# rhinempi/Reflexiv

Measured on AMD Instinct MI355X. Metric: k-mers/sec (extract+count+filter; wall-clock to final contigs beside it), higher is better.
Workload: dtype u64; 1 GPU; synthetic 5 Gbp in all (5 Gbp per GPU x 1), E.coli-like genome 4640000 bp (1078x), PE150, k=31, -cover 30, 0.5% substitutions; reads_per_gpu=33333334, kmer_instances_per_gpu=4000000080, distinct_kmers=352952250, kmers_kept=4639950, parallelism=1 GPU

## Files before the change

### reflexiv_amd/csrc/rfx_count_sk.hip

```cpp
#include "rfx_internal.h"
#include "rfx_device.h"
#include "rfx_count.h"
#include <algorithm>
#include <cmath>

using namespace rfxd;
using namespace rfxc;

namespace {


constexpr int SKT = 1024;

__device__ __forceinline__ uint32_t mmer_key(uint32_t canon) { return __umul24(canon, 0x9E3779u) + canon; }

template <int W, bool RUNLOOP, int SEG = 16, class F>
__device__ __forceinline__ void seg_runs(const ReadSrc &s, int nk_r, int sgm, const uint64_t (&w)[3], F &&emit,
                                         uint64_t *hi_out, uint64_t *lo_out, uint32_t *wm_lds = nullptr, uint32_t *nx_out = nullptr) {
    static_assert(SEG == 16 || SEG == 32, "segment");
    constexpr int PK = SEG;
    constexpr bool MERGE = SEG == 32;
    static_assert(!MERGE || RUNLOOP, "the merged cut walks the run-start bits");
    constexpr int NM = PK + W - 1;
    static_assert(NM + SK_M - 1 <= 64, "the segment's bases lie in (hi, lo)");
    const int p0 = sgm * PK;
    int v = nk_r - p0;
    v = v > PK ? PK : v;
    if constexpr (MERGE) {
        v = v < 0 ? 0 : v;
        if (!__any(v > 0)) return;
    } else if (v <= 0) return;
    const int sh = 2 * ((s.fc + p0) & 31);
    const uint64_t hi = sh ? (w[0] << sh) | (w[1] >> (64 - sh)) : w[0];
    const uint64_t lo = sh ? (w[1] << sh) | (w[2] >> (64 - sh)) : w[1];
    *hi_out = hi; *lo_out = lo;
    constexpr int M2 = 2 * SK_M;
    const uint32_t mmask = (1u << M2) - 1;
    uint32_t val[NM];
    static_assert(SK_M == 13 && NM <= 50, "positions below");
    const uint64_t rhi = revcomp(lo, 32), rlo = revcomp(hi, 32);
    const uint32_t FW[4] = {(uint32_t)(hi >> 32), (uint32_t)hi, (uint32_t)(lo >> 32), (uint32_t)lo};
    const uint32_t RW[4] = {(uint32_t)(rhi >> 32), (uint32_t)rhi, (uint32_t)(rlo >> 32), (uint32_t)rlo};
    auto cut = [&](const uint32_t (&Wd)[4], const int pos) __attribute__((always_inline)) -> uint32_t {
        const int wi = pos >> 4, off = 2 * (pos & 15);
        if (off + M2 <= 32) return (Wd[wi] >> (32 - M2 - off)) & mmask;
        return __builtin_amdgcn_alignbit(Wd[wi], Wd[wi < 3 ? wi + 1 : 3], 32 - off) >> (32 - M2);
    };
#pragma unroll
    for (int j = 0; j < NM; j++) {
        const uint32_t fm = cut(FW, j), rm = cut(RW, 64 - SK_M - j);
        val[j] = mmer_key(fm < rm ? fm : rm);
    }
    uint32_t wm[PK];
    if constexpr (W >= PK - 1) {
#pragma unroll
        for (int j = W - 2; j >= 0; j--) val[j] = val[j] < val[j + 1] ? val[j] : val[j + 1];
#pragma unroll
        for (int j = W + 1; j < NM; j++) val[j] = val[j] < val[j - 1] ? val[j] : val[j - 1];
        wm[0] = val[0];
#pragma unroll
        for (int i = 1; i < PK; i++) wm[i] = val[i] < val[W + i - 1] ? val[i] : val[W + i - 1];
    } else {
        uint32_t sfx[NM], pfx[NM];
#pragma unroll
        for (int j = NM - 1; j >= 0; j--)
            sfx[j] = (j % W == W - 1 || j == NM - 1) ? val[j] : (val[j] < sfx[j + 1] ? val[j] : sfx[j + 1]);
#pragma unroll
        for (int j = 0; j < NM; j++) pfx[j] = (j % W == 0) ? val[j] : (val[j] < pfx[j - 1] ? val[j] : pfx[j - 1]);
#pragma unroll
        for (int i = 0; i < PK; i++) wm[i] = sfx[i] < pfx[i + W - 1] ? sfx[i] : pfx[i + W - 1];
    }
    if constexpr (!RUNLOOP) {
        uint32_t cur = wm[0];
        int start = 0;
#pragma unroll
        for (int i = 1; i < PK; i++) {
            if (i < v && (wm[i] != cur || (PK > 16 && i - start == 16))) {
                emit(start, i - start, cur);
                cur = wm[i]; start = i;
            }
        }
        emit(start, v - start, cur);
        return;
    }
    uint32_t starts = 1u;
#pragma unroll
    for (int i = 1; i < PK; i++) starts |= (uint32_t)(wm[i] != wm[i - 1]) << i;
    const uint32_t vmask = v ? 0xffffffffu >> (32 - v) : 0u;
    starts &= vmask;
    if constexpr (PK > 16) {
        uint32_t cov = starts;
        cov |= cov << 1; cov |= cov << 2; cov |= cov << 4; cov |= cov << 8;
        const uint32_t unc = ~cov & vmask;
        starts |= unc & (0u - unc);
    }
    int vend = v;
    if constexpr (MERGE) {
        const int lane = (int)(threadIdx.x & 63);
        const uint32_t rest = starts & (starts - 1);
        const int b = !v ? 0 : rest ? __ffs((int)rest) - 1 : v;
        const int t = v == PK ? __clz((int)starts) + 1 : 0;
        const uint32_t hk = wm[0], tk = wm[PK - 1];
        const uint32_t hk_n = (uint32_t)__shfl_down((int)hk, 1);
        const uint32_t pk_n = (uint32_t)__shfl_down((int)(((uint32_t)(lo >> 32) & 0xFFFFFFC0u) | (uint32_t)b), 1);
        const uint32_t tk_p = (uint32_t)__shfl_up((int)tk, 1);
        const int t_p = __shfl_up(t, 1);
        const bool next_same = lane < 63 && sgm + 1 < s.segs, prev_same = lane > 0 && sgm > 0;
        const int b_n = (int)(pk_n & 31u);
        if (nx_out) *nx_out = next_same ? pk_n & 0xFFFFFFC0u : 0u;
        if (next_same && t > 0 && b_n > 0 && tk == hk_n) vend = v + (16 - t < b_n ? 16 - t : b_n);
        if (prev_same && t_p > 0 && b > 0 && tk_p == hk) {
            const int a = 16 - t_p < b ? 16 - t_p : b;
            if (a > 0) starts = (starts & ~1u) | (a < b ? 1u << a : 0u);
        }
    }
    if (wm_lds) {
#pragma unroll
        for (int i = 0; i < PK; i++) wm_lds[i * SKT + threadIdx.x] = wm[i];
    }
    uint32_t m0 = wm[0], m1 = wm[1], m2 = wm[2], m3 = wm[3], m4 = wm[4], m5 = wm[5], m6 = wm[6], m7 = wm[7], m8 = wm[8],
             m9 = wm[9], m10 = wm[10], m11 = wm[11], m12 = wm[12], m13 = wm[13], m14 = wm[14], m15 = wm[15];
    if (!wm_lds)
        asm("" : "+v"(m0), "+v"(m1), "+v"(m2), "+v"(m3), "+v"(m4), "+v"(m5), "+v"(m6), "+v"(m7), "+v"(m8), "+v"(m9), "+v"(m10),
                 "+v"(m11), "+v"(m12), "+v"(m13), "+v"(m14), "+v"(m15));
    constexpr int UP = PK > 16 ? 16 : 0;
    uint32_t n0 = wm[UP + 0], n1 = wm[UP + 1], n2 = wm[UP + 2], n3 = wm[UP + 3], n4 = wm[UP + 4], n5 = wm[UP + 5], n6 = wm[UP + 6],
             n7 = wm[UP + 7], n8 = wm[UP + 8], n9 = wm[UP + 9], n10 = wm[UP + 10], n11 = wm[UP + 11], n12 = wm[UP + 12],
             n13 = wm[UP + 13], n14 = wm[UP + 14], n15 = wm[UP + 15];
    if (!wm_lds && PK > 16)
        asm("" : "+v"(n0), "+v"(n1), "+v"(n2), "+v"(n3), "+v"(n4), "+v"(n5), "+v"(n6), "+v"(n7), "+v"(n8), "+v"(n9), "+v"(n10),
                 "+v"(n11), "+v"(n12), "+v"(n13), "+v"(n14), "+v"(n15));
    while (starts) {
        const int i0 = __ffs((int)starts) - 1;
        starts &= starts - 1;
        const int i1 = starts ? __ffs((int)starts) - 1 : vend;
        uint32_t key;
        if (wm_lds) {
            key = wm_lds[i0 * SKT + threadIdx.x];
        } else {
            const bool b0 = i0 & 1, b1 = i0 & 2, b2 = i0 & 4, b3 = i0 & 8;
            const uint32_t a0 = b0 ? m1 : m0, a1 = b0 ? m3 : m2, a2 = b0 ? m5 : m4, a3 = b0 ? m7 : m6, a4 = b0 ? m9 : m8,
                           a5 = b0 ? m11 : m10, a6 = b0 ? m13 : m12, a7 = b0 ? m15 : m14;
            const uint32_t c0 = b1 ? a1 : a0, c1 = b1 ? a3 : a2, c2 = b1 ? a5 : a4, c3 = b1 ? a7 : a6;
            const uint32_t d0 = b2 ? c1 : c0, d1 = b2 ? c3 : c2;
            key = b3 ? d1 : d0;
            if constexpr (PK > 16) {
                const uint32_t e0 = b0 ? n1 : n0, e1 = b0 ? n3 : n2, e2 = b0 ? n5 : n4, e3 = b0 ? n7 : n6, e4 = b0 ? n9 : n8,
                               e5 = b0 ? n11 : n10, e6 = b0 ? n13 : n12, e7 = b0 ? n15 : n14;
                const uint32_t f0 = b1 ? e1 : e0, f1 = b1 ? e3 : e2, f2 = b1 ? e5 : e4, f3 = b1 ? e7 : e6;
                const uint32_t g0 = b2 ? f1 : f0, g1 = b2 ? f3 : f2;
                const uint32_t ku = b3 ? g1 : g0;
                key = (i0 & 16) ? ku : key;
            }
        }
        emit(i0, i1 - i0, key);
    }
}

__device__ __forceinline__ uint64_t mmer_hash64(uint32_t canon) { return kmer_hash((uint64_t)canon); }

__device__ __forceinline__ unsigned sk_digit(uint32_t canon, const Level &lv) {
    const uint64_t h = mmer_hash64(canon);
    if (lv.n_owners > 0) {
        const unsigned o = (unsigned)__umul64hi(h, (uint64_t)lv.n_owners);
        return lv.sub_bits ? (o << lv.sub_bits) | ((uint32_t)((h << OWNER_BITS) >> 32) >> (32 - lv.sub_bits)) : o;
    }
    return rec_digit((uint32_t)((h << OWNER_BITS) >> 32), 0, lv.bits);
}

constexpr int SKD = 8;

template <int W, bool DESC, bool WIDE = false>
__global__ __launch_bounds__(SKT) void k_sk_hist(ReadSrc s, Level lv, uint64_t *__restrict__ blockhist,
                                                 uint32_t *__restrict__ desc) {
    __shared__ uint32_t h[1 << MAX_BITS];
    __shared__ uint32_t wmcol[DESC ? PK * SKT : 1];
    const int nb = lv.n_owners > 0 ? lv.n_owners : (1 << lv.bits);
    for (int i = threadIdx.x; i < nb; i += SKT) h[i] = 0;
    __syncthreads();
    const int64_t stride = (int64_t)gridDim.x * SKT;
    const int64_t dq = stride / s.segs;
    const int dr = (int)(stride - dq * s.segs);
    int64_t g = (int64_t)blockIdx.x * SKT + threadIdx.x;
    SegPos q;
    q.r = g / s.segs;
    q.sgm = (int)(g - q.r * s.segs);
    for (; g < s.n_threads; g += stride) {
        uint64_t w[3], hi, lo;
        seg_load(s, q, w);
        if constexpr (DESC) {
            uint32_t mask = 0, nr = 0;
            uint32_t own[2] = {0, 0};
            seg_runs<W, true>(s, read_nk<WIDE>(s, q.r), q.sgm, w, [&](int i0, int, uint32_t canon) {
                const uint64_t h64 = mmer_hash64(canon);
                const uint32_t hdr = (uint32_t)((h64 << OWNER_BITS) >> 32);
                const unsigned d = lv.n_owners > 0 ? (unsigned)__umul64hi(h64, (uint64_t)lv.n_owners) : rec_digit(hdr, 0, lv.bits);
                atomicAdd(&h[d], 1u);
                if (nr < (uint32_t)SKD) {
                    desc[(int64_t)(1 + nr) * s.n_threads + g] = hdr;
                    if (nr < 4) own[0] |= d << (8 * nr); else own[1] |= d << (8 * (nr - 4));
                }
                mask |= 1u << i0; nr++;
            }, &hi, &lo, wmcol);
            desc[g] = mask | (nr << 16);
            if (lv.n_owners > 0) {
                desc[(int64_t)(1 + SKD) * s.n_threads + g] = own[0];
                desc[(int64_t)(2 + SKD) * s.n_threads + g] = own[1];
            }
        } else {
            seg_runs<W, false>(s, read_nk<WIDE>(s, q.r), q.sgm, w, [&](int, int, uint32_t canon) { atomicAdd(&h[sk_digit(canon, lv)], 1u); }, &hi, &lo);
        }
        q.r += dq; q.sgm += dr;
        if (q.sgm >= s.segs) { q.sgm -= s.segs; q.r++; }
    }
    __syncthreads();
    for (int i = threadIdx.x; i < nb; i += SKT) blockhist[(int64_t)i * gridDim.x + blockIdx.x] = h[i];
}

constexpr int SKB = 8, SKA = 4;
template <int W, bool DESC, bool WIDE = false>
__global__ __launch_bounds__(SKT, WIDE ? 4 : 8) void k_sk_scatter(ReadSrc s, Level lv, const uint64_t *__restrict__ scanned,
                                                              std::conditional_t<WIDE, WRec, Rec> *__restrict__ out,
                                                              const uint32_t *__restrict__ desc) {
    using RT = std::conditional_t<WIDE, WRec, Rec>;
    extern __shared__ __attribute__((aligned(32))) unsigned char sk_smem[];
    const int nb = lv.n_owners > 0 ? lv.n_owners : (1 << lv.bits);
#define buf ((RT *)sk_smem)
#define tail ((unsigned long long *)(sk_smem + (size_t)nb * SKB * sizeof(RT)))
#define head (tail + nb)
    for (int i = threadIdx.x; i < nb; i += SKT) tail[i] = head[i] = scanned[(int64_t)i * gridDim.x + blockIdx.x];
    __syncthreads();
    auto drain = [&](bool final) __attribute__((always_inline)) {
        for (int d = threadIdx.x / SKB; d < nb; d += SKT / SKB) {
            const int j = threadIdx.x % SKB;
            const unsigned long long h = head[d], t = tail[d];
            unsigned long long e, nh;
            if (t - h > (unsigned long long)SKB) { e = h + SKB; nh = t; }
            else {
                e = final ? t : (t & ~(unsigned long long)(SKA - 1));
                if (e < h) e = h;
                nh = e;
            }
            const unsigned long long g = h + j;
            if (g < e) out[g] = buf[(size_t)d * SKB + (g & (SKB - 1))];
            if (j == 0) head[d] = nh;
        }
    };
    const int64_t stride = (int64_t)gridDim.x * SKT;
    const int64_t dq = stride / s.segs;
    const int dr = (int)(stride - dq * s.segs);
    const int64_t g0 = (int64_t)blockIdx.x * SKT;
    int64_t g = g0 + threadIdx.x;
    SegPos q;
    q.r = g / s.segs;
    q.sgm = (int)(g - q.r * s.segs);
    for (int64_t gb = g0; gb < s.n_threads; gb += stride, g += stride) {
        if (g < s.n_threads) {
            uint64_t w[3], hi = 0, lo = 0;
            seg_load(s, q, w);
            auto put = [&](int i0, int n, uint32_t hdr, unsigned d) __attribute__((always_inline)) {
                RT r;
                if constexpr (WIDE) {
                    const uint64_t *gw = s.words + q.r * s.wpr;
                    const int p = s.fc - s.wfl + q.sgm * PK + i0;
                    const int wi = p >> 5, sft = 2 * (p & 31), last = s.wpr - 1;
                    const uint64_t a0 = gw[wi < last ? wi : last], a1 = gw[wi + 1 < last ? wi + 1 : last];
                    const uint64_t a2 = gw[wi + 2 < last ? wi + 2 : last], a3 = gw[wi + 3 < last ? wi + 3 : last];
                    r.b0 = sft ? (a0 << sft) | (a1 >> (64 - sft)) : a0;
                    r.b1 = sft ? (a1 << sft) | (a2 >> (64 - sft)) : a1;
                    r.b2 = sft ? (a2 << sft) | (a3 >> (64 - sft)) : a2;
                    r.hd = ((uint64_t)(n - 1) << 32) | (uint64_t)hdr;
                } else {
                    const int sft = 2 * i0;
                    r.w0 = sft ? (hi << sft) | (lo >> (64 - sft)) : hi;
                    r.w1 = ((lo << sft) & 0xFFFFFFF000000000ULL) | ((uint64_t)(n - 1) << 32) | (uint64_t)hdr;
                }
                const unsigned long long pos = atomicAdd(&tail[d], 1ULL);
                if (pos - head[d] < (unsigned long long)SKB) buf[(size_t)d * SKB + (pos & (SKB - 1))] = r;
                else out[pos] = r;
            };
            auto recompute = [&]() __attribute__((always_inline)) {
                seg_runs<W, true>(s, read_nk<WIDE>(s, q.r), q.sgm, w, [&](int i0, int n, uint32_t canon) {
                    const uint64_t h = mmer_hash64(canon);
                    const unsigned d = lv.n_owners > 0 ? (unsigned)__umul64hi(h, (uint64_t)lv.n_owners)
                                                       : rec_digit((uint32_t)((h << OWNER_BITS) >> 32), 0, lv.bits);
                    put(i0, n, (uint32_t)((h << OWNER_BITS) >> 32), d);
                }, &hi, &lo);
            };
            if constexpr (DESC) {
                const uint32_t m = desc[g];
                const uint32_t nr = m >> 16;
                if (nr > (uint32_t)SKD) {
                    recompute();
                } else if (nr) {
                    const int p0 = q.sgm * PK;
                    int v = read_nk<WIDE>(s, q.r) - p0;
                    v = v > PK ? PK : v;
                    const int sh = 2 * ((s.fc + p0) & 31);
                    hi = sh ? (w[0] << sh) | (w[1] >> (64 - sh)) : w[0];
                    lo = sh ? (w[1] << sh) | (w[2] >> (64 - sh)) : w[1];
                    uint32_t hd[SKD];
#pragma unroll
                    for (int r = 0; r < SKD; r++) hd[r] = (uint32_t)r < nr ? desc[(int64_t)(1 + r) * s.n_threads + g] : 0u;
                    uint32_t own[2] = {0, 0};
                    if (lv.n_owners > 0) {
                        own[0] = desc[(int64_t)(1 + SKD) * s.n_threads + g];
                        own[1] = desc[(int64_t)(2 + SKD) * s.n_threads + g];
                    }
                    uint32_t starts = m & 0xffffu;
#pragma unroll
                    for (int r = 0; r < SKD; r++) {
                        if (starts) {
                            const int i0 = __ffs((int)starts) - 1;
                            starts &= starts - 1;
                            const int i1 = starts ? __ffs((int)starts) - 1 : v;
                            put(i0, i1 - i0, hd[r], lv.n_owners > 0 ? (own[r >> 2] >> (8 * (r & 3))) & 255u : rec_digit(hd[r], 0, lv.bits));
                        }
                    }
                }
            } else {
                recompute();
            }
            q.r += dq; q.sgm += dr;
            if (q.sgm >= s.segs) { q.sgm -= s.segs; q.r++; }
        }
        __syncthreads();
        drain(false);
        __syncthreads();
    }
    drain(true);
}
#undef buf
#undef tail
#undef head

constexpr int OSE_MIN = 64, OSE_MAX = 256;
constexpr int OS_CSTRIDE = 16;
constexpr int OS_MAXG = 512;
constexpr int OS_HOLES = 3;
struct OneSweep {
    const uint64_t *reg_start;
    const uint32_t *reg_cap;
    unsigned long long *cursor;
    uint64_t *holes;
    int *overflow;
    uint64_t total;
    unsigned long long *tile_counter;
    uint32_t ose, ose_shift;
};

template <int W, int SEG = 16, bool WIDE = false>
__global__ __launch_bounds__(SKT) void k_sk_sample_hist(ReadSrc s, Level lv, int sample, unsigned long long *__restrict__ hist) {
    __shared__ uint32_t h[1 << MAX_BITS];
    const int nb = 1 << lv.bits;
    for (int i = threadIdx.x; i < nb; i += SKT) h[i] = 0;
    __syncthreads();
    const int64_t ntile = (s.n_threads + SKT - 1) / SKT;
    for (int64_t T = (int64_t)blockIdx.x * sample; T < ntile; T += (int64_t)gridDim.x * sample) {
        const int64_t g = T * SKT + threadIdx.x;
        const bool in = g < s.n_threads;
        SegPos q{0, 0};
        int nk_r = 0;
        uint64_t w[3] = {0, 0, 0}, hi, lo;
        if (in) {
            q.r = g / s.segs;
            q.sgm = (int)(g - q.r * s.segs);
            seg_load<SEG>(s, q, w);
            nk_r = read_nk<WIDE>(s, q.r);
        }
        if (SEG == 32 || in)
            seg_runs<W, SEG == 32, SEG>(s, nk_r, q.sgm, w, [&](int, int, uint32_t canon) { atomicAdd(&h[sk_digit(canon, lv)], 1u); }, &hi, &lo);
    }
    __syncthreads();
    for (int i = threadIdx.x; i < nb; i += SKT) if (h[i]) atomicAdd(&hist[i], (unsigned long long)h[i]);
}

__global__ __launch_bounds__(1024) void k_plan_regions(const unsigned long long *__restrict__ hist, int nb, double scale, int G, int cap_pct,
                                                       double tiles,
                                                       uint64_t *__restrict__ reg_start, uint32_t *__restrict__ reg_cap,
                                                       unsigned long long *__restrict__ cursor, unsigned long long *__restrict__ totals) {
    __shared__ uint64_t caps[1 << MAX_BITS];
    __shared__ unsigned long long busiest;
    __shared__ uint32_t ose_s;
    const int d = threadIdx.x;
    if (d == 0) busiest = 0;
    __syncthreads();
    if (d < nb) atomicMax(&busiest, hist[d]);
    __syncthreads();
    if (d == 0) {
        const double per_tile = (double)busiest * scale / tiles;
        ose_s = per_tile <= 16.0 ? 64u : per_tile <= 32.0 ? 128u : per_tile <= 64.0 ? 256u : 0u;
    }
    __syncthreads();
    const uint32_t E = ose_s ? ose_s : OSE_MIN;
    if (d < nb) {
        const double c = (double)hist[d];
        const double est = c * scale;
        double room = (est + 6.0 * scale * sqrt(c + 1.0) + est / 64.0 + 1024.0) * (double)cap_pct / 100.0;
        uint64_t cap = (uint64_t)room + (uint64_t)G * OS_HOLES * E;
        cap = (cap + E - 1) / E * E;
        if (cap > 0xFFFFFF00ULL) cap = 0xFFFFFF00ULL / E * E;
        caps[d] = cap;
        reg_cap[d] = (uint32_t)cap;
    }
    __syncthreads();
    if (threadIdx.x == 0) {
        uint64_t at = 0;
        for (int i = 0; i < nb; i++) { reg_start[i] = at; cursor[(size_t)i * OS_CSTRIDE] = at; at += caps[i]; }
        reg_start[nb] = at;
        totals[0] = at + E;
        totals[1] = 0;
        totals[2] = ose_s;
    }
}

template <int SEG, bool WIDE> struct OsGeo {
    static constexpr int T = SEG > 16 && !WIDE ? 512 : SKT;
};
template <int W, bool WIDE = false, int SEG = 16>
__global__ __launch_bounds__((OsGeo<SEG, WIDE>::T), 4) void k_sk_onesweep(ReadSrc s, Level lv, OneSweep os,
                                                               std::conditional_t<WIDE, WRec, Rec> *__restrict__ out) {
    using RT = std::conditional_t<WIDE, WRec, Rec>;
    constexpr int SKT = OsGeo<SEG, WIDE>::T;
    extern __shared__ __attribute__((aligned(32))) unsigned char sk_smem[];
    const int nb = 1 << lv.bits;
#define buf ((RT *)sk_smem)
#define tail ((uint32_t *)(sk_smem + (size_t)nb * SKB * sizeof(RT)))
#define head (tail + nb)
#define cstart (tail + 2 * nb)
#define cbase (tail + 3 * nb)
#define nbase (tail + 4 * nb)
#define pbase (tail + 5 * nb)
    constexpr uint32_t DUMP = 0xFFFFFFFFu;
    const uint32_t OSE = os.ose, OSH = os.ose_shift;
    const uint64_t dump_at = os.total - OSE;
    auto extent_of = [&](unsigned long long b) __attribute__((always_inline)) -> uint32_t {
        return b + OSE <= dump_at ? (uint32_t)(b >> OSH) : DUMP;
    };
    auto grab = [&](int d) __attribute__((always_inline)) -> uint32_t {
        return extent_of(atomicAdd(&os.cursor[(size_t)d * OS_CSTRIDE], (unsigned long long)OSE));
    };
    auto phys = [&](uint32_t v, uint32_t cs, uint32_t cb, uint32_t nx) __attribute__((always_inline)) -> uint64_t {
        const uint32_t o = v - cs;
        const uint32_t b = o < (uint32_t)OSE ? cb : nx;
        return (b == DUMP ? dump_at : (uint64_t)b << OSH) + (o & (OSE - 1));
    };
    constexpr uint32_t NONE = 0xFFFFFFFEu;
    for (int i = threadIdx.x; i < nb; i += SKT) {
        tail[i] = 0; head[i] = 0; cstart[i] = 0;
        cbase[i] = grab(i);
        nbase[i] = grab(i);
        pbase[i] = grab(i);
    }
    __syncthreads();
    constexpr int LPB = SEG > 16 || WIDE ? 4 : SKB;
    auto drain = [&](bool final) __attribute__((always_inline)) {
#pragma nounroll
        for (int d = threadIdx.x / LPB; d < nb; d += SKT / LPB) {
            const int j = threadIdx.x % LPB;
            const uint32_t h = head[d], t = tail[d], cs = cstart[d], cb = cbase[d], nx = nbase[d];
            uint32_t e, nh;
            if (t - h > (uint32_t)SKB) { e = h + SKB; nh = t; }
            else {
                e = final ? t : (t & ~(uint32_t)(SKA - 1));
                if (e < h) e = h;
                nh = e;
            }
#pragma unroll
            for (int q = 0; q < SKB / LPB; q++) {
                const uint32_t g = h + j + q * LPB;
                if (g < e) l2_store_stream(out + phys(g, cs, cb, nx), buf[(size_t)d * SKB + (g & (SKB - 1))]);
            }
            if (j == 0) {
                head[d] = nh;
                if (nh - cs >= (uint32_t)OSE) {
                    const uint32_t b2 = pbase[d];
                    cstart[d] = cs + OSE; cbase[d] = nx; nbase[d] = final && b2 == NONE ? DUMP : b2; pbase[d] = NONE;
                }
            }
        }
    };
    __shared__ long long tile_lds[2];
    const int64_t ntile = (s.n_threads + SKT - 1) / SKT;
    const int my_d = (int)threadIdx.x;
    int64_t T = blockIdx.x;
    auto fetch = [&](int64_t tile, SegPos &q, int &nk_r, uint64_t (&w)[3]) __attribute__((always_inline)) {
        const int64_t g = tile * SKT + threadIdx.x;
        const int64_t gc = g < s.n_threads ? g : s.n_threads - 1;
        q.r = gc / s.segs;
        q.sgm = (int)(gc - q.r * s.segs);
        seg_load<SEG>(s, q, w);
        nk_r = read_nk<WIDE>(s, q.r);
    };
    int64_t T1 = (int64_t)gridDim.x + blockIdx.x;
    SegPos qn{0, 0};
    int nkn = 0;
    uint64_t wn[3] = {0, 0, 0};
    if (T < ntile) fetch(T, qn, nkn, wn);
    asm volatile("" : "+v"(wn[0]), "+v"(wn[1]), "+v"(wn[2]), "+v"(nkn));
    for (int rnd = 0; T < ntile; rnd++) {
        const bool in = T * SKT + threadIdx.x < s.n_threads;
        SegPos q{in ? qn.r : 0, in ? qn.sgm : 0};
        int nk_r = in ? nkn : 0;
        uint64_t w[3] = {in ? wn[0] : 0, in ? wn[1] : 0, in ? wn[2] : 0}, hi = 0, lo = 0;
        uint32_t past = 0;
        unsigned long long t_raw = 0, req_raw = 0;
        const bool ask = my_d < nb && pbase[my_d] == NONE;
        if (ask) req_raw = atomicAdd(&os.cursor[(size_t)my_d * OS_CSTRIDE], (unsigned long long)OSE);
        fetch(T1, qn, nkn, wn);
        if (threadIdx.x == SKT - 1) t_raw = atomicAdd(os.tile_counter, 1ULL);
        if (SEG == 32 || in) {
            seg_runs<W, true, SEG>(s, nk_r, q.sgm, w, [&](int i0, int n, uint32_t canon) {
                const uint64_t hh = mmer_hash64(canon);
                const uint32_t hdr = (uint32_t)((hh << OWNER_BITS) >> 32);
                const unsigned d = lv.n_owners > 0 ? (((unsigned)__umul64hi(hh, (uint64_t)lv.n_owners) << lv.sub_bits) | (hdr >> (32 - lv.sub_bits)))
                                                   : rec_digit(hdr, 0, lv.bits);
                RT r;
                if constexpr (WIDE) {
                    const uint64_t *gw = s.words + q.r * s.wpr;
                    const int p = s.fc - s.wfl + q.sgm * SEG + i0;
                    const int wi = p >> 5, sft = 2 * (p & 31), last = s.wpr - 1;
                    const uint64_t a0 = gw[wi < last ? wi : last], a1 = gw[wi + 1 < last ? wi + 1 : last];
                    const uint64_t a2 = gw[wi + 2 < last ? wi + 2 : last], a3 = gw[wi + 3 < last ? wi + 3 : last];
                    r.b0 = sft ? (a0 << sft) | (a1 >> (64 - sft)) : a0;
                    r.b1 = sft ? (a1 << sft) | (a2 >> (64 - sft)) : a1;
                    r.b2 = sft ? (a2 << sft) | (a3 >> (64 - sft)) : a2;
                    r.hd = ((uint64_t)(n - 1) << 32) | (uint64_t)hdr;
                } else {
                    const uint32_t d0 = (uint32_t)(hi >> 32), d1 = (uint32_t)hi, d2 = (uint32_t)(lo >> 32), d3 = (uint32_t)lo;
                    const uint32_t e0 = d0 >> 1, e1 = __builtin_amdgcn_alignbit(d0, d1, 1), e2 = __builtin_amdgcn_alignbit(d1, d2, 1);
                    const uint32_t e3 = __builtin_amdgcn_alignbit(d2, d3, 1), e4 = __builtin_amdgcn_alignbit(d3, past, 1);
                    const bool up = i0 >= 16;
                    const uint32_t a0 = up ? e1 : e0, a1 = up ? e2 : e1, a2 = up ? e3 : e2, a3 = up ? e4 : e3;
                    const uint32_t sh = 31u - 2u * ((uint32_t)i0 & 15u);
                    const uint32_t w0h = __builtin_amdgcn_alignbit(a0, a1, sh), w0l = __builtin_amdgcn_alignbit(a1, a2, sh);
                    const uint32_t w1h = (__builtin_amdgcn_alignbit(a2, a3, sh) & 0xFFFFFFF0u) | (uint32_t)(n - 1);
                    r.w0 = ((uint64_t)w0h << 32) | w0l;
                    r.w1 = ((uint64_t)w1h << 32) | (uint64_t)hdr;
                }
                const uint32_t pos = atomicAdd(&tail[d], 1u);
                if (pos - head[d] < (uint32_t)SKB) buf[(size_t)d * SKB + (pos & (SKB - 1))] = r;
                else {
                    const uint32_t cs = cstart[d];
                    if (pos - cs < 2u * OSE) out[phys(pos, cs, cbase[d], nbase[d])] = r;
                    else { os.overflow[0] = 1; os.overflow[1] = 1; }
                }
            }, &hi, &lo, nullptr, &past);
        }
        asm volatile("" : "+v"(wn[0]), "+v"(wn[1]), "+v"(wn[2]), "+v"(nkn), "+v"(t_raw), "+v"(req_raw));
        if (threadIdx.x == SKT - 1) tile_lds[rnd & 1] = 2LL * (long long)gridDim.x + (long long)t_raw;
        if (ask) pbase[my_d] = extent_of(req_raw);
        __syncthreads();
        drain(false);
        T = T1;
        T1 = tile_lds[rnd & 1];
        __syncthreads();
    }
    drain(true);
    __syncthreads();
    for (int d = threadIdx.x; d < nb; d += SKT) {
        const uint32_t used = tail[d] - cstart[d], cb = cbase[d], nx = nbase[d], px = pbase[d];
        uint64_t *hl = os.holes + ((size_t)d * gridDim.x + blockIdx.x) * OS_HOLES;
        hl[0] = cb != DUMP && used < OSE ? ((((uint64_t)cb << OSH) + used) << 16) | (uint64_t)(OSE - used) : 0;
        hl[1] = nx != DUMP ? (((uint64_t)nx << OSH) << 16) | (uint64_t)OSE : 0;
        hl[2] = px != DUMP && px != NONE ? (((uint64_t)px << OSH) << 16) | (uint64_t)OSE : 0;
    }
}
#undef buf
#undef tail
#undef head
#undef cstart
#undef cbase
#undef nbase
#undef pbase

constexpr int FH_T = 1024;
template <class RT>
__global__ __launch_bounds__(FH_T) void k_fix_holes(OneSweep os, int G, RT *__restrict__ out, uint64_t *__restrict__ seg_begin,
                                                   uint64_t *__restrict__ seg_end, unsigned long long *__restrict__ totals) {
    constexpr int NHMAX = 2048;
    static_assert(NHMAX >= OS_HOLES * OS_MAXG && NHMAX % FH_T == 0, "holes per bucket");
    constexpr int NWMAX = NHMAX * OSE_MAX / 32;
    __shared__ uint32_t hstart[NHMAX], hoff[NHMAX + 1];
    __shared__ uint32_t bitmap[NWMAX];
    __shared__ uint32_t wsum[FH_T / 64];
    const int d = blockIdx.x;
    const int NH = OS_HOLES * G;
    const uint64_t base = os.reg_start[d];
    const unsigned long long alloc = os.cursor[(size_t)d * OS_CSTRIDE] - base;
    if (alloc > (unsigned long long)os.reg_cap[d]) {
        if (threadIdx.x == 0) { seg_begin[d] = base; seg_end[d] = base; *os.overflow = 1; }
        return;
    }
    auto block_excl_scan = [&](uint32_t v, uint32_t *total) __attribute__((always_inline)) -> uint32_t {
        const int lane = threadIdx.x & 63, wave = threadIdx.x >> 6;
        uint32_t x = v;
#pragma unroll
        for (int o = 1; o < 64; o <<= 1) { const uint32_t y = __shfl_up(x, o, 64); if (lane >= o) x += y; }
        if (lane == 63) wsum[wave] = x;
        __syncthreads();
        uint32_t b = 0, tot = 0;
        for (int i = 0; i < FH_T / 64; i++) { const uint32_t sv = wsum[i]; if (i < wave) b += sv; tot += sv; }
        __syncthreads();
        *total = tot;
        return b + x - v;
    };
    constexpr int HPT = NHMAX / FH_T;
    uint32_t hs[HPT], hl[HPT];
    uint32_t mine = 0;
#pragma unroll
    for (int r = 0; r < HPT; r++) {
        const int t = threadIdx.x * HPT + r;
        const uint64_t x = t < NH ? os.holes[(size_t)d * NH + t] : 0;
        hl[r] = (uint32_t)(x & 0xFFFFu);
        hs[r] = hl[r] ? (uint32_t)((x >> 16) - base) : 0u;
        mine += hl[r];
    }
    uint32_t H;
    block_excl_scan(mine, &H);
    const uint32_t size = (uint32_t)alloc - H;
    const uint32_t nw = (H + 31) / 32;
    const uint32_t wpt = (nw + FH_T - 1) / FH_T;
    for (uint32_t i = threadIdx.x; i < nw; i += FH_T) bitmap[i] = 0;
    __syncthreads();
    uint32_t fill[HPT], fsum = 0;
#pragma unroll
    for (int r = 0; r < HPT; r++) {
        fill[r] = hs[r] < size ? (hs[r] + hl[r] <= size ? hl[r] : size - hs[r]) : 0u;
        fsum += fill[r];
        for (uint32_t p = hs[r] + fill[r]; p < hs[r] + hl[r]; p++) atomicOr(&bitmap[(p - size) >> 5], 1u << ((p - size) & 31));
    }
    uint32_t F;
    uint32_t fo = block_excl_scan(fsum, &F);
#pragma unroll
    for (int r = 0; r < HPT; r++) {
        const int t = threadIdx.x * HPT + r;
        hstart[t] = hs[r]; hoff[t] = fo; fo += fill[r];
    }
    if (threadIdx.x == 0) hoff[NHMAX] = F;
    __syncthreads();
    auto valid_word = [&](uint32_t w) __attribute__((always_inline)) -> uint32_t {
        if (w >= nw) return 0u;
        const uint32_t lim = H - w * 32 >= 32 ? 0xFFFFFFFFu : (1u << (H - w * 32)) - 1u;
        return ~bitmap[w] & lim;
    };
    uint32_t vsum = 0;
    for (uint32_t r = 0; r < wpt; r++) vsum += (uint32_t)__popc(valid_word(threadIdx.x * wpt + r));
    uint32_t V;
    uint32_t vo = block_excl_scan(vsum, &V);
    for (uint32_t r = 0; r < wpt; r++) {
        const uint32_t w = threadIdx.x * wpt + r;
        uint32_t m = valid_word(w);
        while (m) {
            const int b = __ffs((int)m) - 1;
            m &= m - 1;
            const uint32_t i = vo++;
            if (i < F) {
                int lo = 0, hi = NHMAX;
                while (hi - lo > 1) { const int mid = (lo + hi) >> 1; if (hoff[mid] <= i) lo = mid; else hi = mid; }
                out[base + hstart[lo] + (i - hoff[lo])] = out[base + size + w * 32 + b];
            }
        }
    }
    if (threadIdx.x == 0) {
        seg_begin[d] = base; seg_end[d] = base + size;
        atomicAdd(&totals[1], (unsigned long long)size);
        if (V != F) *os.overflow = 2;
    }
}

}

namespace rfx {

#define RFX_SK_W_CASES(X) X(9) X(10) X(11) X(12) X(13) X(14) X(15) X(16) X(17) X(18)
template <bool DESC, bool WIDE = false, class... Args>
static int launch_sk_hist(rfx_ctx *ctx, int W, dim3 grid, Args... args) {
    if constexpr (WIDE) {
        if (W == 18) RFX_LAUNCH((k_sk_hist<18, DESC, true>), grid, dim3(SKT), 0, args...);
        else RFX_LAUNCH((k_sk_hist<19, DESC, true>), grid, dim3(SKT), 0, args...);
        return RFX_OK;
    }
    switch (W) {
#define X(w) case w: RFX_LAUNCH((k_sk_hist<w, DESC>), grid, dim3(SKT), 0, args...); break;
        RFX_SK_W_CASES(X)
#undef X
        default: RFX_LAUNCH((k_sk_hist<19, DESC>), grid, dim3(SKT), 0, args...); break;
    }
    return RFX_OK;
}

template <int W, bool DESC, bool WIDE, class... Args>
static int launch_sk_scatter_w(rfx_ctx *ctx, dim3 grid, size_t lds, Args... args) {
    RFX_HIP(hipFuncSetAttribute((const void *)k_sk_scatter<W, DESC, WIDE>, hipFuncAttributeMaxDynamicSharedMemorySize, (int)lds));
    RFX_LAUNCH((k_sk_scatter<W, DESC, WIDE>), grid, dim3(SKT), lds, args...);
    return RFX_OK;
}
template <bool DESC, bool WIDE, class... Args>
static int launch_sk_scatter(rfx_ctx *ctx, int W, dim3 grid, size_t lds, Args... args) {
    if constexpr (WIDE) {
        if (W == 18) return launch_sk_scatter_w<18, DESC, true>(ctx, grid, lds, args...);
        return launch_sk_scatter_w<19, DESC, true>(ctx, grid, lds, args...);
    } else {
        switch (W) {
#define X(w) case w: return launch_sk_scatter_w<w, DESC, false>(ctx, grid, lds, args...);
            RFX_SK_W_CASES(X)
#undef X
            default: return launch_sk_scatter_w<19, DESC, false>(ctx, grid, lds, args...);
        }
    }
}

template <bool WIDE>
int records_from_reads(rfx_ctx *ctx, const ReadSrc &rsrc, const Level &lv, bool use_ws, int ws_slot,
                       std::conditional_t<WIDE, WRec, Rec> *d_dst, int64_t cap_dst, uint64_t *d_seg_off,
                       std::conditional_t<WIDE, WRec, Rec> **out_recs, int64_t *n_recs,
                       const char *hn, const char *pn) {
    using Rec = std::conditional_t<WIDE, WRec, ::Rec>;
    const int nb = lv.n_owners > 0 ? lv.n_owners : (1 << lv.bits);
    const int W = rsrc.k - SK_M + 1;
    const size_t sk_lds = (size_t)nb * (SKB * sizeof(Rec) + 16);
    const int per_cu = sk_lds <= 80 * 1024 ? 8 : 1;
    const unsigned G = (unsigned)std::max<int64_t>(1, std::min<int64_t>(ceil_div(rsrc.n_threads, SKT), (int64_t)ctx->num_cu * per_cu));
    DevBuf bh, scanned;
    RFX_ALLOC(bh, uint64_t, (size_t)nb * G);
    RFX_ALLOC(scanned, uint64_t, (size_t)nb * G + 1);
    uint32_t *desc = nullptr;
    const bool want_desc = lv.n_owners <= 64 && count_tuning().sk_desc;
    if (want_desc) desc = (uint32_t *)ctx->ws_get(use_ws && ws_slot == 1 ? 0 : 1, (size_t)(3 + SKD) * 4 * (size_t)rsrc.n_threads);
    {
        ScopedTimer t(ctx, hn);
        if (desc) RFX_TRY((launch_sk_hist<true, WIDE>(ctx, W, dim3(G), rsrc, lv, bh.as<uint64_t>(), desc)));
        else RFX_TRY((launch_sk_hist<false, WIDE>(ctx, W, dim3(G), rsrc, lv, bh.as<uint64_t>(), (uint32_t *)nullptr)));
    }
    RFX_TRY(exclusive_scan_u64(ctx, bh.as<uint64_t>(), scanned.as<uint64_t>(), (int64_t)nb * G));
    RFX_TRY(bin_offsets(ctx, scanned.as<uint64_t>(), nb, (int64_t)G, d_seg_off));
    uint64_t R = 0;
    RFX_HIP(hipMemcpyAsync(&R, scanned.as<uint64_t>() + (size_t)nb * G, 8, hipMemcpyDeviceToHost, ctx->stream));
    RFX_TRY(sync_checked(ctx));
    *n_recs = (int64_t)R;
    Rec *dst = d_dst;
    if (use_ws) {
        dst = (Rec *)ctx->ws_get(ws_slot, (size_t)R * sizeof(Rec));
        if (!dst) { ctx->last_error = "workspace allocation failed"; return RFX_E_HIP; }
    } else if (!dst || (int64_t)R > cap_dst) {
        return RFX_E_CAP;
    }
    {
        ScopedTimer t(ctx, pn);
        if (desc) RFX_TRY((launch_sk_scatter<true, WIDE>(ctx, W, dim3(G), sk_lds, rsrc, lv, scanned.as<uint64_t>(), dst, (const uint32_t *)desc)));
        else RFX_TRY((launch_sk_scatter<false, WIDE>(ctx, W, dim3(G), sk_lds, rsrc, lv, scanned.as<uint64_t>(), dst, (const uint32_t *)nullptr)));
    }
    *out_recs = dst;
    return RFX_OK;
}

template <bool WIDE>
int records_onesweep(rfx_ctx *ctx, const ReadSrc &rsrc_in, const Level &lv, int ws_slot, uint64_t *d_seg_begin,
                     uint64_t *d_seg_end, std::conditional_t<WIDE, WRec, Rec> **out_recs, int64_t *n_recs, bool *done,
                     const char *hn, const char *pn, std::conditional_t<WIDE, WRec, Rec> *d_dst, int64_t cap_dst) {
    using Rec = std::conditional_t<WIDE, WRec, ::Rec>;
    const CountTuning tune = count_tuning();
    *done = false;
    const int nb = 1 << lv.bits;
    const int W = rsrc_in.k - SK_M + 1;
    const bool seg32 = !WIDE && nb <= 512;
    ReadSrc rsrc = rsrc_in;
    if (seg32) {
        rsrc.segs = rsrc.nk > 0 ? (rsrc.nk + 31) / 32 : 1;
        rsrc.n_threads = rsrc.n_reads * rsrc.segs;
    }
    const int OST = seg32 ? OsGeo<32, false>::T : SKT;
    const int64_t ntile = ceil_div(rsrc.n_threads, OST);
    const int64_t ntile_s = ceil_div(rsrc.n_threads, SKT);
    const int per_cu = WIDE ? 1 : 2;
    const int G = (int)std::max<int64_t>(1, std::min<int64_t>(std::min<int64_t>(OS_MAXG, (int64_t)ctx->num_cu * per_cu),
                                                                std::max<int64_t>(std::min<int64_t>(ntile, 64), ntile / 32)));
    int sample = 32;
    if (ntile_s < 64 * (int64_t)sample) sample = (int)std::max<int64_t>(1, ntile_s / 64);
    const int64_t n_sampled = ceil_div(ntile_s, sample);
    const int cap_pct = tune.sk_onesweep_cap;
    DevBuf hist, reg_start, reg_cap, cursor, totals, holes;
    RFX_HIP(hist.alloc((size_t)nb * 8 + 16, ctx->stream));
    RFX_ALLOC(reg_start, uint64_t, nb + 1);
    RFX_ALLOC(reg_cap, uint32_t, nb);
    RFX_ALLOC(cursor, unsigned long long, (size_t)nb * OS_CSTRIDE);
    RFX_HIP(totals.alloc(24, ctx->stream));
    RFX_ALLOC(holes, uint64_t, (size_t)nb * OS_HOLES * G);
    RFX_HIP(hipMemsetAsync(hist.p, 0, (size_t)nb * 8 + 16, ctx->stream));
    int *d_overflow = (int *)(hist.as<unsigned long long>() + nb);
    {
        ScopedTimer t(ctx, hn);
        const dim3 gs((unsigned)std::min<int64_t>(n_sampled, (int64_t)ctx->num_cu * 8));
        if constexpr (WIDE) {
            if (W == 18) RFX_LAUNCH((k_sk_sample_hist<18, 16, true>), gs, dim3(SKT), 0, rsrc, lv, sample, hist.as<unsigned long long>());
            else RFX_LAUNCH((k_sk_sample_hist<19, 16, true>), gs, dim3(SKT), 0, rsrc, lv, sample, hist.as<unsigned long long>());
        } else switch (W) {
#define X(w) case w: if (seg32) RFX_LAUNCH((k_sk_sample_hist<w, 32>), gs, dim3(SKT), 0, rsrc, lv, sample, hist.as<unsigned long long>()); \
                     else RFX_LAUNCH((k_sk_sample_hist<w>), gs, dim3(SKT), 0, rsrc, lv, sample, hist.as<unsigned long long>()); break;
            RFX_SK_W_CASES(X)
            default: X(19)
#undef X
        }
        RFX_LAUNCH(k_plan_regions, dim3(1), dim3(1024), 0, hist.as<unsigned long long>(), nb,
                   (double)ntile_s / (double)n_sampled, G, cap_pct, (double)ntile, reg_start.as<uint64_t>(), reg_cap.as<uint32_t>(),
                   cursor.as<unsigned long long>(), totals.as<unsigned long long>());
    }
    unsigned long long h_tot[3] = {0, 0, 0};
    RFX_HIP(hipMemcpyAsync(h_tot, totals.p, 24, hipMemcpyDeviceToHost, ctx->stream));
    RFX_TRY(sync_checked(ctx));
    const uint32_t ose = (uint32_t)h_tot[2];
    if (ose == 0) {
        if (tune.trace) fprintf(stderr, "one-sweep level 1: not tried (the sample puts too much on one bucket)\n");
        return RFX_OK;
    }
    int ose_shift = 0;
    while ((1u << ose_shift) < ose) ose_shift++;
    Rec *dst = d_dst;
    if (d_dst) {
        if ((int64_t)h_tot[0] > cap_dst) { *n_recs = (int64_t)h_tot[0]; return RFX_E_CAP; }
    } else {
        dst = (Rec *)ctx->ws_get(ws_slot, (size_t)h_tot[0] * sizeof(Rec));
        if (!dst) { ctx->last_error = "workspace allocation failed"; return RFX_E_HIP; }
    }
    const OneSweep os{reg_start.as<uint64_t>(), reg_cap.as<uint32_t>(), cursor.as<unsigned long long>(), holes.as<uint64_t>(), d_overflow,
                      (uint64_t)h_tot[0], hist.as<unsigned long long>() + nb + 1, ose, (uint32_t)ose_shift};
    const size_t lds = (size_t)nb * (SKB * sizeof(Rec) + 24);
    {
        ScopedTimer t(ctx, pn);
        if constexpr (WIDE) {
            if (W == 18) {
                RFX_HIP(hipFuncSetAttribute((const void *)k_sk_onesweep<18, true>, hipFuncAttributeMaxDynamicSharedMemorySize, (int)lds));
                RFX_LAUNCH((k_sk_onesweep<18, true>), dim3((unsigned)G), dim3(SKT), lds, rsrc, lv, os, dst);
            } else {
                RFX_HIP(hipFuncSetAttribute((const void *)k_sk_onesweep<19, true>, hipFuncAttributeMaxDynamicSharedMemorySize, (int)lds));
                RFX_LAUNCH((k_sk_onesweep<19, true>), dim3((unsigned)G), dim3(SKT), lds, rsrc, lv, os, dst);
            }
        } else {
            switch (W) {
#define X(w) case w: if (seg32) { \
                         RFX_HIP(hipFuncSetAttribute((const void *)k_sk_onesweep<w, false, 32>, hipFuncAttributeMaxDynamicSharedMemorySize, (int)lds)); \
                         RFX_LAUNCH((k_sk_onesweep<w, false, 32>), dim3((unsigned)G), dim3(OST), lds, rsrc, lv, os, dst); \
                     } else { \
                         RFX_HIP(hipFuncSetAttribute((const void *)k_sk_onesweep<w>, hipFuncAttributeMaxDynamicSharedMemorySize, (int)lds)); \
                         RFX_LAUNCH((k_sk_onesweep<w>), dim3((unsigned)G), dim3(SKT), lds, rsrc, lv, os, dst); \
                     } break;
                RFX_SK_W_CASES(X)
                default: X(19)
#undef X
            }
        }
        RFX_LAUNCH(k_fix_holes<Rec>, dim3((unsigned)nb), dim3(FH_T), 0, os, G, dst, d_seg_begin, d_seg_end,
                   totals.as<unsigned long long>());
    }
    int h_flag[2] = {0, 0};
    RFX_HIP(hipMemcpyAsync(h_tot, totals.p, 16, hipMemcpyDeviceToHost, ctx->stream));
    RFX_HIP(hipMemcpyAsync(h_flag, d_overflow, 8, hipMemcpyDeviceToHost, ctx->stream));
    RFX_TRY(sync_checked(ctx));
    const int h_over = h_flag[0];
    if (h_flag[1]) ctx->timing["stat_l1_void_rounds"].launches += 1;
    if (tune.trace)
        fprintf(stderr, "one-sweep level 1: %llu records in regions of %llu (sample 1/%d, %d workgroups, extents of %u)%s\n", h_tot[1], h_tot[0], sample, G, ose,
                h_over ? " -- a region overflowed: two passes instead" : "");
    if (h_over == 2) { ctx->last_error = "one-sweep level 1: holes and tail records do not balance"; return RFX_E_STATE; }
    if (h_over) return RFX_OK;
    *out_recs = dst;
    *n_recs = (int64_t)h_tot[1];
    ctx->timing["stat_records"].launches += (int64_t)h_tot[1];
    *done = true;
    return RFX_OK;
}

int count_reads_superkmer(rfx_ctx *ctx, const ReadStore *reads, int min_cov, int max_cov, int twin,
                          uint64_t *d_out_keys, int32_t *d_out_counts, int64_t cap, int64_t *out_n,
                          int64_t *out_distinct, bool pair_out) {
    ctx->timing.clear();
    ReadSrc rsrc = make_read_src(reads);
    const int64_t n = instances_of(reads, rsrc);
    if (out_n) *out_n = 0;
    if (out_distinct) *out_distinct = 0;
    if (n <= 0) return RFX_OK;
    std::vector<int> bits;
    plan_levels(n, true, bits, 16384.0);
    Level lv{};
    lv.bits = bits[0];
    StageArena stage_arena(ctx, ((size_t)64 << 20) + (size_t)n / 8);
    DevBuf segA, segB;
    RFX_ALLOC(segA, uint64_t, (size_t)(1 << lv.bits) + 1);
    Rec *recs = nullptr;
    int64_t R = 0;
    bool swept = false;
    DevBuf segE;
    if (bits.size() >= 2 && sweep_level1(count_tuning(), rsrc.n_threads)) {
        RFX_ALLOC(segE, uint64_t, 1 << lv.bits);
        RFX_TRY(records_onesweep(ctx, rsrc, lv, 0, segA.as<uint64_t>(), segE.as<uint64_t>(), &recs, &R, &swept, "hist1", "part1"));
    }
    if (!swept) RFX_TRY(records_from_reads(ctx, rsrc, lv, true, 0, nullptr, 0, segA.as<uint64_t>(), &recs, &R, "hist1", "part1"));
    return count_records_levels(ctx, recs, R, 0, bits, 1, lv.bits, &segA, &segB, (int64_t)1 << lv.bits, reads->k,
                                min_cov, max_cov, twin, d_out_keys, d_out_counts, cap, out_n, out_distinct, pair_out,
                                swept ? segE.as<uint64_t>() : nullptr);
}

int bucket_records_by_owner(rfx_ctx *ctx, const ReadStore *reads, int n_owners, void *d_out, int64_t cap_records,
                            int64_t *d_owner_off, int64_t *h_owner_off, int64_t *out_n_records) {
    StageArena stage_arena(ctx, (size_t)256 << 20);
    if (n_owners < 1 || n_owners > 64 || !superkmer_enabled(reads->k)) return RFX_E_ARG;
    ReadSrc rsrc = make_read_src(reads);
    if (out_n_records) *out_n_records = 0;
    if (rsrc.nk <= 0 || reads->n_reads <= 0) return zero_owner_offsets(ctx, n_owners, d_owner_off, h_owner_off);
    Level lv{};
    lv.n_owners = n_owners;
    Rec *recs = nullptr;
    int64_t R = 0;
    int st = records_from_reads(ctx, rsrc, lv, false, 0, (Rec *)d_out, cap_records,
                                reinterpret_cast<uint64_t *>(d_owner_off), &recs, &R, "hist1", "part1");
    if (out_n_records) *out_n_records = R;
    if (st != RFX_OK) return st;
    if (h_owner_off) {
        RFX_HIP(hipMemcpyAsync(h_owner_off, d_owner_off, (size_t)(n_owners + 1) * 8, hipMemcpyDeviceToHost, ctx->stream));
        RFX_TRY(sync_checked(ctx));
    }
    return RFX_OK;
}

template <class RT>
static __global__ __launch_bounds__(1024) void k_close_gaps(RT *__restrict__ recs, const uint64_t *__restrict__ seg_begin,
                                                     const uint64_t *__restrict__ seg_end, int S, uint64_t *__restrict__ out_begin,
                                                     uint64_t *__restrict__ out_end, int *__restrict__ fault) {
    __shared__ uint64_t slo[512], dlo[512], spre[513], dpre[513];
    const int o = blockIdx.x;
    const uint64_t *sb = seg_begin + (size_t)o * S, *se = seg_end + (size_t)o * S;
    if (threadIdx.x == 0) {
        uint64_t R = 0;
        for (int i = 0; i < S; i++) R += se[i] - sb[i];
        const uint64_t cut = sb[0] + R;
        spre[0] = dpre[0] = 0;
        for (int i = 0; i < S; i++) {
            const uint64_t lo = sb[i] > cut ? sb[i] : cut;
            slo[i] = lo;
            spre[i + 1] = spre[i] + (se[i] > lo ? se[i] - lo : 0);
            uint64_t g0 = se[i], g1 = i + 1 < S ? sb[i + 1] : se[i];
            if (g1 > cut) g1 = cut;
            dlo[i] = g0;
            dpre[i + 1] = dpre[i] + (g1 > g0 ? g1 - g0 : 0);
        }
        if (spre[S] != dpre[S]) *fault = 1;
        if (blockIdx.y == 0) { out_begin[o] = sb[0]; out_end[o] = cut; }
    }
    __syncthreads();
    const uint64_t M = spre[S] < dpre[S] ? spre[S] : dpre[S];
    for (uint64_t k = (uint64_t)blockIdx.y * blockDim.x + threadIdx.x; k < M; k += (uint64_t)gridDim.y * blockDim.x) {
        int i = 0, j = 0;
        for (int st = S >> 1; st > 0; st >>= 1) {
            if (spre[i + st] <= k) i += st;
            if (dpre[j + st] <= k) j += st;
        }
        recs[dlo[j] + (k - dpre[j])] = recs[slo[i] + (k - spre[i])];
    }
}

template <bool WIDE>
static int owner_sweep(rfx_ctx *ctx, const ReadSrc &rsrc, int n_owners, void *d_out, int64_t cap_records, int64_t *h_begin,
                       int64_t *h_end, int64_t *out_n_records, bool *done) {
    using RT = std::conditional_t<WIDE, WRec, Rec>;
    *done = false;
    if (rsrc.nk <= 0 || rsrc.n_reads <= 0 || !sweep_level1(count_tuning(), rsrc.n_threads)) return RFX_OK;
    StageArena stage_arena(ctx, (size_t)256 << 20);
    int obits = 0;
    while ((1 << obits) < n_owners) obits++;
    Level lv{};
    lv.n_owners = n_owners;
    lv.sub_bits = 9 - obits;
    lv.bits = 9;
    const int nb = 1 << lv.bits, S = 1 << lv.sub_bits;
    DevBuf segB, segE, ob, oe, flt;
    RFX_ALLOC(segB, uint64_t, nb + 1);
    RFX_ALLOC(segE, uint64_t, nb);
    RFX_ALLOC(ob, uint64_t, n_owners);
    RFX_ALLOC(oe, uint64_t, n_owners);
    RFX_HIP(flt.alloc(4, ctx->stream));
    RFX_HIP(hipMemsetAsync(flt.p, 0, 4, ctx->stream));
    RT *recs = nullptr;
    int64_t R = 0;
    bool swept = false;
    int st = records_onesweep<WIDE>(ctx, rsrc, lv, 0, segB.as<uint64_t>(), segE.as<uint64_t>(), &recs, &R, &swept, "hist1", "part1",
                                    (RT *)d_out, cap_records);
    if (out_n_records) *out_n_records = R;
    if (st != RFX_OK || !swept) return st;
    {
        ScopedTimer t(ctx, "part1");
        RFX_LAUNCH(k_close_gaps<RT>, dim3((unsigned)n_owners, 16), dim3(1024), 0, recs, segB.as<uint64_t>(),
                   segE.as<uint64_t>(), S, ob.as<uint64_t>(), oe.as<uint64_t>(), flt.as<int>());
    }
    int h_fault = 0;
    static_assert(sizeof(int64_t) == sizeof(uint64_t), "offsets");
    RFX_HIP(hipMemcpyAsync(h_begin, ob.p, (size_t)n_owners * 8, hipMemcpyDeviceToHost, ctx->stream));
    RFX_HIP(hipMemcpyAsync(h_end, oe.p, (size_t)n_owners * 8, hipMemcpyDeviceToHost, ctx->stream));
    RFX_HIP(hipMemcpyAsync(&h_fault, flt.p, 4, hipMemcpyDeviceToHost, ctx->stream));
    RFX_TRY(sync_checked(ctx));
    if (h_fault) { ctx->last_error = "owner sweep: gaps and tail records do not balance"; return RFX_E_STATE; }
    *done = true;
    return RFX_OK;
}

int bucket_records_by_owner_sweep(rfx_ctx *ctx, const ReadStore *reads, int n_owners, void *d_out, int64_t cap_records,
                                  int64_t *h_begin, int64_t *h_end, int64_t *out_n_records, bool *done) {
    *done = false;
    if (n_owners < 1 || n_owners > 64 || !superkmer_enabled(reads->k)) return RFX_E_ARG;
    return owner_sweep<false>(ctx, make_read_src(reads), n_owners, d_out, cap_records, h_begin, h_end, out_n_records, done);
}

ReadSrc wide_read_src(const uint64_t *d_words, int64_t n_reads, int wpr, int64_t nk, int k, int fc,
                      const uint32_t *d_read_len, int ec) {
    ReadSrc s{};
    const int c = (k & 1) ? 31 : 30;
    s.words = d_words; s.n_reads = n_reads; s.wpr = wpr;
    s.wfl = (k - c) / 2;
    s.fc = fc + s.wfl; s.k = c;
    s.nk = (int)nk;
    s.segs = s.nk > 0 ? (s.nk + PK - 1) / PK : 1;
    s.n_threads = s.n_reads * s.segs;
    s.len_arr = d_read_len; s.ec = ec;
    return s;
}

int bucket_wide_records_by_owner(rfx_ctx *ctx, const uint64_t *d_words, int64_t n_reads, int wpr, int64_t nk, int k, int fc,
                                 int n_owners, void *d_out, int64_t cap_records, int64_t *d_owner_off, int64_t *h_owner_off,
                                 int64_t *out_n_records, const uint32_t *d_read_len, int ec) {
    StageArena stage_arena(ctx, (size_t)256 << 20);
    if (n_owners < 1 || n_owners > 64 || k < 33 || k > 63) return RFX_E_ARG;
    if (out_n_records) *out_n_records = 0;
    if (nk <= 0 || n_reads <= 0) return zero_owner_offsets(ctx, n_owners, d_owner_off, h_owner_off);
    ReadSrc rsrc = wide_read_src(d_words, n_reads, wpr, nk, k, fc, d_read_len, ec);
    Level lv{};
    lv.n_owners = n_owners;
    WRec *recs = nullptr;
    int64_t R = 0;
    const int st = records_from_reads<true>(ctx, rsrc, lv, false, 0, (WRec *)d_out, cap_records,
                                            reinterpret_cast<uint64_t *>(d_owner_off), &recs, &R, "hist1", "part1");
    if (out_n_records) *out_n_records = R;
    if (st != RFX_OK) return st;
    if (h_owner_off) {
        RFX_HIP(hipMemcpyAsync(h_owner_off, d_owner_off, (size_t)(n_owners + 1) * 8, hipMemcpyDeviceToHost, ctx->stream));
        RFX_TRY(sync_checked(ctx));
    }
    return RFX_OK;
}

int bucket_wide_records_by_owner_sweep(rfx_ctx *ctx, const uint64_t *d_words, int64_t n_reads, int wpr, int64_t nk, int k, int fc,
                                       int n_owners, void *d_out, int64_t cap_records, int64_t *h_begin, int64_t *h_end,
                                       int64_t *out_n_records, bool *done, const uint32_t *d_read_len, int ec) {
    *done = false;
    if (n_owners < 1 || n_owners > 64 || k < 33 || k > 63) return RFX_E_ARG;
    if (nk <= 0 || n_reads <= 0) return RFX_OK;
    return owner_sweep<true>(ctx, wide_read_src(d_words, n_reads, wpr, nk, k, fc, d_read_len, ec), n_owners, d_out, cap_records, h_begin, h_end,
                             out_n_records, done);
}

template decltype(records_from_reads<false>) records_from_reads<false>;
template decltype(records_from_reads<true>) records_from_reads<true>;
template decltype(records_onesweep<false>) records_onesweep<false>;
template decltype(records_onesweep<true>) records_onesweep<true>;

}
```

Before: 212.5 billion k-mers/s.

## Replace hole bitmap with per-extent used counts in fix-holes compaction

The compaction kernel that fills holes in each bucket's output region no longer marks every tail hole slot in a shared-memory bitmap with per-element atomics. Each tail extent now records its used prefix with one atomicMin. Valid source elements are then located by a prefix scan over extents and a branchless binary search. The copy loop is unrolled four ways with vectorized loads and stores, and holes are validated, with overflow flagged on malformed input. This removes per-slot atomics, the popcount/ffs bit walk and serial per-thread work, at the cost of more shared-memory scan arrays and two binary searches per moved element.

```diff
diff --git a/reflexiv_amd/csrc/rfx_count_sk.hip b/reflexiv_amd/csrc/rfx_count_sk.hip
--- a/reflexiv_amd/csrc/rfx_count_sk.hip
+++ b/reflexiv_amd/csrc/rfx_count_sk.hip
@@ -1,6 +1,7 @@
 #include "rfx_internal.h"
 #include "rfx_device.h"
 #include "rfx_count.h"
+#include "rfx_fix_holes.h"
 #include <algorithm>
 #include <cmath>
 
@@ -579,13 +580,14 @@
 __global__ __launch_bounds__(FH_T) void k_fix_holes(OneSweep os, int G, RT *__restrict__ out, uint64_t *__restrict__ seg_begin,
                                                    uint64_t *__restrict__ seg_end, unsigned long long *__restrict__ totals) {
     constexpr int NHMAX = 2048;
-    static_assert(NHMAX >= OS_HOLES * OS_MAXG && NHMAX % FH_T == 0, "holes per bucket");
-    constexpr int NWMAX = NHMAX * OSE_MAX / 32;
-    __shared__ uint32_t hstart[NHMAX], hoff[NHMAX + 1];
-    __shared__ uint32_t bitmap[NWMAX];
+    static_assert(NHMAX >= OS_HOLES * OS_MAXG + 1 && NHMAX % FH_T == 0 && (NHMAX & (NHMAX - 1)) == 0, "holes per bucket");
+    static_assert(OSE_MAX <= 0xFFFF, "a hole's length is filed in 16 bits");
+    __shared__ uint32_t hstart[NHMAX], hoff[NHMAX];
+    __shared__ uint32_t used[NHMAX], soff[NHMAX];
     __shared__ uint32_t wsum[FH_T / 64];
     const int d = blockIdx.x;
     const int NH = OS_HOLES * G;
+    const uint32_t sh = os.ose_shift, E = os.ose;
     const uint64_t base = os.reg_start[d];
     const unsigned long long alloc = os.cursor[(size_t)d * OS_CSTRIDE] - base;
     if (alloc > (unsigned long long)os.reg_cap[d]) {
@@ -612,55 +614,65 @@
     for (int r = 0; r < HPT; r++) {
         const int t = threadIdx.x * HPT + r;
         const uint64_t x = t < NH ? os.holes[(size_t)d * NH + t] : 0;
-        hl[r] = (uint32_t)(x & 0xFFFFu);
-        hs[r] = hl[r] ? (uint32_t)((x >> 16) - base) : 0u;
+        if (!fh_hole(x, base, alloc, sh, &hs[r], &hl[r])) *os.overflow = 2;
         mine += hl[r];
     }
     uint32_t H;
     block_excl_scan(mine, &H);
+    if ((unsigned long long)H > alloc) {
+        if (threadIdx.x == 0) { seg_begin[d] = base; seg_end[d] = base; *os.overflow = 2; }
+        return;
+    }
     const uint32_t size = (uint32_t)alloc - H;
-    const uint32_t nw = (H + 31) / 32;
-    const uint32_t wpt = (nw + FH_T - 1) / FH_T;
-    for (uint32_t i = threadIdx.x; i < nw; i += FH_T) bitmap[i] = 0;
+    const uint32_t e0 = fh_first_extent(size, sh), NE = fh_tail_extents(size, (uint32_t)alloc, sh);
+    for (uint32_t i = threadIdx.x; i < (uint32_t)NHMAX; i += FH_T) used[i] = i < NE ? E : 0u;
     __syncthreads();
     uint32_t fill[HPT], fsum = 0;
 #pragma unroll
     for (int r = 0; r < HPT; r++) {
-        fill[r] = hs[r] < size ? (hs[r] + hl[r] <= size ? hl[r] : size - hs[r]) : 0u;
+        fill[r] = fh_fill(hs[r], hl[r], size);
         fsum += fill[r];
-        for (uint32_t p = hs[r] + fill[r]; p < hs[r] + hl[r]; p++) atomicOr(&bitmap[(p - size) >> 5], 1u << ((p - size) & 31));
+        const uint32_t j = (hs[r] >> sh) - e0;
+        if (fill[r] < hl[r] && j < (uint32_t)NHMAX) atomicMin(&used[j], hs[r] & (E - 1));
     }
     uint32_t F;
     uint32_t fo = block_excl_scan(fsum, &F);
+    uint32_t src_n[HPT], ssum = 0;
 #pragma unroll
     for (int r = 0; r < HPT; r++) {
-        const int t = threadIdx.x * HPT + r;
+        const uint32_t t = threadIdx.x * HPT + r;
         hstart[t] = hs[r]; hoff[t] = fo; fo += fill[r];
-    }
-    if (threadIdx.x == 0) hoff[NHMAX] = F;
-    __syncthreads();
-    auto valid_word = [&](uint32_t w) __attribute__((always_inline)) -> uint32_t {
-        if (w >= nw) return 0u;
-        const uint32_t lim = H - w * 32 >= 32 ? 0xFFFFFFFFu : (1u << (H - w * 32)) - 1u;
-        return ~bitmap[w] & lim;
-    };
-    uint32_t vsum = 0;
-    for (uint32_t r = 0; r < wpt; r++) vsum += (uint32_t)__popc(valid_word(threadIdx.x * wpt + r));
+        src_n[r] = t < NE ? fh_sources((e0 + t) << sh, used[t], size) : 0u;
+        ssum += src_n[r];
+    }
     uint32_t V;
-    uint32_t vo = block_excl_scan(vsum, &V);
-    for (uint32_t r = 0; r < wpt; r++) {
-        const uint32_t w = threadIdx.x * wpt + r;
-        uint32_t m = valid_word(w);
-        while (m) {
-            const int b = __ffs((int)m) - 1;
-            m &= m - 1;
-            const uint32_t i = vo++;
-            if (i < F) {
-                int lo = 0, hi = NHMAX;
-                while (hi - lo > 1) { const int mid = (lo + hi) >> 1; if (hoff[mid] <= i) lo = mid; else hi = mid; }
-                out[base + hstart[lo] + (i - hoff[lo])] = out[base + size + w * 32 + b];
+    uint32_t so = block_excl_scan(ssum, &V);
+#pragma unroll
+    for (int r = 0; r < HPT; r++) { soff[threadIdx.x * HPT + r] = so; so += src_n[r]; }
+    __syncthreads();
+    constexpr int FH_U = 4, FH_Q = (int)sizeof(RT) / 16;
+    constexpr uint32_t NOPOS = 0xFFFFFFFFu;
+    const uint32_t n = F < V ? F : V;
+    for (uint32_t i0 = threadIdx.x; i0 < n; i0 += FH_U * FH_T) {
+        l2_v2 v[FH_U][FH_Q];
+        uint32_t src[FH_U], dst[FH_U];
+#pragma unroll
+        for (int u = 0; u < FH_U; u++) {
+            const uint32_t i = i0 + (uint32_t)u * FH_T, ic = i < n ? i : i0;
+            src[u] = fh_source(soff, NHMAX, e0, sh, size, ic);
+            const uint32_t dp = fh_dest(hstart, hoff, NHMAX, ic);
+            dst[u] = i < n ? dp : NOPOS;
+        }
+#pragma unroll
+        for (int u = 0; u < FH_U; u++)
+#pragma unroll
+            for (int q = 0; q < FH_Q; q++) v[u][q] = ((const l2_v2 *)(out + base + src[u]))[q];
+#pragma unroll
+        for (int u = 0; u < FH_U; u++)
+            if (dst[u] != NOPOS) {
+#pragma unroll
+                for (int q = 0; q < FH_Q; q++) ((l2_v2 *)(out + base + dst[u]))[q] = v[u][q];
             }
-        }
     }
     if (threadIdx.x == 0) {
         seg_begin[d] = base; seg_end[d] = base + size;
diff --git a/reflexiv_amd/csrc/rfx_fix_holes.h b/reflexiv_amd/csrc/rfx_fix_holes.h
--- /dev/null
+++ b/reflexiv_amd/csrc/rfx_fix_holes.h
@@ -0,0 +1,50 @@
+#pragma once
+#include <stdint.h>
+
+#ifdef __HIPCC__
+#define FH_INLINE __host__ __device__ __forceinline__
+#define FH_UNROLL _Pragma("unroll")
+#else
+#define FH_INLINE inline
+#define FH_UNROLL
+#endif
+
+FH_INLINE bool fh_hole(uint64_t x, uint64_t base, uint64_t alloc, uint32_t sh, uint32_t *start, uint32_t *len) {
+    const uint64_t l = x & 0xFFFFu, a = x >> 16, E = 1ull << sh;
+    *start = 0; *len = 0;
+    if (l == 0) return true;
+    if (a < base || a - base >= alloc || l > E || ((a - base) & (E - 1)) + l != E) return false;
+    *start = (uint32_t)(a - base); *len = (uint32_t)l;
+    return true;
+}
+
+FH_INLINE uint32_t fh_fill(uint32_t hs, uint32_t hl, uint32_t size) {
+    return hs < size ? (hl <= size - hs ? hl : size - hs) : 0u;
+}
+
+FH_INLINE uint32_t fh_sources(uint32_t ebeg, uint32_t used, uint32_t size) {
+    const uint32_t b = ebeg > size ? ebeg : size, e = ebeg + used;
+    return e > b ? e - b : 0u;
+}
+
+FH_INLINE uint32_t fh_first_extent(uint32_t size, uint32_t sh) { return size >> sh; }
+FH_INLINE uint32_t fh_tail_extents(uint32_t size, uint32_t alloc, uint32_t sh) { return (alloc >> sh) - (size >> sh); }
+
+FH_INLINE int fh_find(const uint32_t *off, int n, uint32_t i) {
+    int lo = 0;
+    FH_UNROLL
+    for (int b = 15; b >= 0; b--)
+        if ((n >> 1) >> b && off[lo + (1 << b)] <= i) lo += 1 << b;
+    return lo;
+}
+
+FH_INLINE uint32_t fh_dest(const uint32_t *hstart, const uint32_t *hoff, int n, uint32_t i) {
+    const int j = fh_find(hoff, n, i);
+    return hstart[j] + (i - hoff[j]);
+}
+
+FH_INLINE uint32_t fh_source(const uint32_t *soff, int n, uint32_t e0, uint32_t sh, uint32_t size, uint32_t i) {
+    const int j = fh_find(soff, n, i);
+    const uint32_t ebeg = (e0 + (uint32_t)j) << sh;
+    return (ebeg > size ? ebeg : size) + (i - soff[j]);
+}
```

Result: no change. 214.5 billion k-mers/s, median of 6 (+0.9%).
